# falcon-computing/bwa-flow

Hardware: AMD Instinct MI355X
Metric: million reads/sec (2×150 bp PE) end-to-end align; SW-extend GCUPS at 1/2/4/8 MI355X (higher is better)
Workload: dtype int32

## Files before the change

### bwa-flow_amd/csrc/capi.hip

```cpp
#include <hip/hip_runtime.h>
#include <string.h>

#include <algorithm>
#include <chrono>
#include <cstdio>
#include <mutex>
#include <new>
#include <string>
#include <thread>
#include <vector>

#include "batch_host.h"
#include "ctx.h"
#include "engine.h"
#include "regpost.h"

using namespace bwagpu;

namespace {


__global__ void side_probe_spin(uint64_t ticks) {
  const uint64_t t0 = __builtin_amdgcn_s_memrealtime();
  while (__builtin_amdgcn_s_memrealtime() - t0 < ticks) __builtin_amdgcn_s_sleep(8);
// ... 114 lines not shown
  if (hipGetDeviceCount(&n) != hipSuccess || n <= 0) return BWAGPU_E_NODEVICE;
  if (device < 0 || device >= n) return BWAGPU_E_NODEVICE;
  bwagpu_ctx_t* ctx = new (std::nothrow) bwagpu_ctx_t();
  if (!ctx) return BWAGPU_E_NOMEM;
  std::string why;
  if (!make_opt(opt, &ctx->opt, &why)) {
    delete ctx;
    return BWAGPU_E_INVAL;
  }
  ctx->device = device;
  ctx->opt_b = opt->b;
  ctx->ext_form = set_ext_form(-1);
  ctx->ext_short = ext_short_default();
  ctx->ext_short_fill = ext_short_fill_default();
  ctx->light_pack = light_pack_default();
  *made = ctx;
  HIPC(hipSetDevice(device), "hipSetDevice");
  HIPC(hipMalloc(&ctx->d_ann_off, sizeof(int64_t) * bns->n_seqs), "hipMalloc(ann_offset)");
  HIPC(hipMalloc(&ctx->d_ann_len, sizeof(int32_t) * bns->n_seqs), "hipMalloc(ann_len)");
  HIPC(hipMemcpy(ctx->d_ann_off, bns->ann_offset, sizeof(int64_t) * bns->n_seqs, hipMemcpyHostToDevice),
       "upload ann_offset");
  HIPC(hipMemcpy(ctx->d_ann_len, bns->ann_len, sizeof(int32_t) * bns->n_seqs, hipMemcpyHostToDevice),
       "upload ann_len");
  for (auto& s : ctx->slot) {
    HIPC(hipEventCreate(&s.ev0), "hipEventCreate");
    HIPC(hipEventCreate(&s.ev1), "hipEventCreate");
    HIPC(hipEventCreate(&s.ev2), "hipEventCreate");
    HIPC(hipEventCreate(&s.ev3), "hipEventCreate");
  }
  ctx->ref.l_pac = bns->l_pac;
// ... 138 lines not shown
  HIPC(s.d_heavy.get(a.heavy, nr), "hipMalloc(heavy)");
  HIPC(s.d_redo.get(a.redo, nr), "hipMalloc(redo)");
  HIPC(s.d_rbits.get(a.rbits, nr / 32 + 1), "hipMalloc(rbits)");
  HIPC(s.d_desc.get(a.rdesc, nr), "hipMalloc(desc)");
  HIPC(s.d_schain.get(a.seedchain, ns), "hipMalloc(seedchain)");
  HIPC(s.d_hinfo.get(a.hinfo, nr), "hipMalloc(hinfo)");
  HIPC(s.d_cov.get(a.cov, ns), "hipMalloc(cov)");
  HIPC(s.d_hflag.get(a.hflag, ns), "hipMalloc(hflag)");
  HIPC(s.d_colent.get(a.colent, ns), "hipMalloc(colent)");
  HIPC(s.d_longc.get(a.longc, nc), "hipMalloc(longc)");
  HIPC(s.d_qh.get(a.qh, kQHWords), "hipMalloc(qh)");
  HIPC(s.d_sorth.get(a.sorth, kSortWords), "hipMalloc(sorth)");
  HIPC(s.d_stasks.get(a.stasks, n_tasks), "hipMalloc(stasks)");
  HIPC(s.d_ftask.get(a.ftask, n_tasks), "hipMalloc(ftask)");
  HIPC(s.d_ftaskR.get(a.ftaskR, n_tasks), "hipMalloc(ftaskR)");
  HIPC(s.d_mat.get(a.mat, (size_t)std::max<int64_t>(1 << 20, 16 * (int64_t)ns)), "hipMalloc(mat)");
  a.mat_words = (int64_t)(s.d_mat.cap / sizeof(uint64_t));
  static const int ext_prefetch = [] {
    const char* e = getenv("BWAGPU_EXT_PREFETCH");
    return e ? std::max(0, atoi(e)) : 0;
  }();
  a.ext_prefetch = ext_prefetch;
  static const int risky_first = [] {
    const char* e = getenv("BWAGPU_LIGHT_RISKY_FIRST");
    return e && e[0] == '1';
  }();
  a.risky_first = risky_first;
  static const int emu_strict = [] {
    const char* e = getenv("BWAGPU_EMU_STRICT");
    return !(e && e[0] == '0');
// ... 514 lines not shown
  if (k == BWAGPU_NUM_SLOTS || !ctx->dev_scratch[k].d_ctr.p) return fail(ctx, BWAGPU_E_INVAL, "no device-entry batch on this stream");
  HIPC(hipStreamSynchronize(st), "hipStreamSynchronize");
  int32_t c[SPC_WORDS];
  HIPC(hipMemcpy(c, ctx->dev_scratch[k].d_ctr.p, sizeof c, hipMemcpyDeviceToHost), "hipMemcpy(ctr)");
  out[0] = c[SPC_SHORT_N];
  for (int r = 0; r < 2; ++r) {
    const int l = r * kSpecBins;
    out[1 + 4 * r] = c[SPC_LCNT + l];
    out[2 + 4 * r] = c[SPC_LLONG + l];
    out[3 + 4 * r] = c[SPC_RCNT + l];
    out[4 + 4 * r] = c[SPC_RLONG + l];
  }
  return BWAGPU_OK;
}

int bwagpu_ctx_row_bound(bwagpu_ctx_t* ctx, int on) {
  if (!ctx) return BWAGPU_E_INVAL;
  const int prev = ctx->opt.row_bound;
  if (on >= 0) ctx->opt.row_bound = on ? 1 : 0;
  return prev;
}

int bwagpu_debug_ext_kernel(bwagpu_ctx_t* ctx, int32_t lq_max) {
  if (!ctx || lq_max < 1 || lq_max > BWAGPU_MAX_READ_LEN) return BWAGPU_E_INVAL;
  return ext_kernel_for(ctx->opt, ctx->ext_form, tb_bytes_for(ctx->opt, lq_max));
}

int bwagpu_prof_start(bwagpu_ctx_t* ctx, int max_launches) {
  if (!ctx || max_launches < 0) return BWAGPU_E_INVAL;
  HIPC(hipSetDevice(ctx->device), "hipSetDevice");
// ... 51 lines not shown
```

### bwa-flow_amd/csrc/ctx.h

```cpp
#pragma once
#include <hip/hip_runtime.h>
#include <stdint.h>

#include <algorithm>
#include <atomic>
#include <chrono>
#include <mutex>
#include <string>
#include <type_traits>
#include <vector>

#include "bwagpu.h"
#include "chain.h"
#include "engine.h"
#include "rescue.h"
#include "seed.h"
#include "stage_host.h"
#include "task_host.h"

namespace bwagpu {

inline std::atomic<int64_t> g_live_bufs{0}, g_live_bytes{0};

template <bool kPinned>
// ... 35 lines not shown
  }
  template <class T>
  T* as() const { return (T*)p; }
};
using DevBuf = GrowBuf<false>;
using HostBuf = GrowBuf<true>;
static_assert(!std::is_copy_constructible<DevBuf>::value, "a copy would free the buffer twice");

struct Slot {
  hipStream_t stream = nullptr;
  std::once_flag stream_once;
  hipError_t stream_err = hipSuccess;
  hipEvent_t ev0 = nullptr, ev1 = nullptr, ev2 = nullptr, ev3 = nullptr;
  DevBuf d_in, d_win, d_srt, d_prog, d_desc, d_out, d_n, d_stats, d_lists, d_counts;
  DevBuf d_cread, d_ext, d_tasks, d_ctr, d_regpos, d_skipf, d_heavy, d_redo, d_rbits;
  DevBuf d_schain, d_hinfo, d_mat, d_cov, d_hflag, d_colent, d_qh, d_longc, d_sorth, d_stasks, d_ftask, d_ftaskR;
  SpecStreams spec;
  bool side_chosen = false;
  HostBuf h_in, h_out, h_n, h_stats;
  HostBuf h_dense, h_off;
  DevBuf d_off;
  size_t in_rco = 0, in_cso = 0;
  bool slot_view = false;
  bool busy = false;
  bool has_results = false;
  bool kept = false;
  std::vector<int32_t> keep_rco, keep_cso;
  int32_t n_reads = 0, n_chains = 0, n_seeds = 0;
  std::chrono::steady_clock::time_point t_submit;
  bwagpu_stats_t last{};
  int64_t h2d = 0, d2h = 0;
// ... 30 lines not shown
  using Slot = bwagpu::Slot;
  int device = 0;
  std::mutex side_mu;
  std::vector<hipStream_t> callers, side_graveyard;
  bwagpu::DevOpt opt{};
  bwagpu::DevRef ref{};
  bool own_pac = false;
  void* d_pac = nullptr;
  int64_t* d_ann_off = nullptr;
  int32_t* d_ann_len = nullptr;
  int watchdog_ms = 10000;
  int ext_form = 0;
  int ext_short = 0;
  int light_pack = 0;
  int ext_short_fill = 0;
  Slot slot[BWAGPU_NUM_SLOTS];
  hipStream_t dev_stream[BWAGPU_NUM_SLOTS] = {};
  Slot dev_scratch[BWAGPU_NUM_SLOTS];
  DevBuf ex_tasks, ex_list, ex_q, ex_t, ex_res, ex_stats;
  DevBuf a2_tasks, a2_q, a2_t, a2_out, a2_scratch, a2_lists, a2_counts, a2_boff;
  DevBuf r2_tasks, r2_q, r2_out, r2_cig, r2_md, r2_lists, r2_z, r2_stats;
  DevBuf r2d_keys, r2d_lists, r2d_tab, r2d_z, r2d_sums;
  HostBuf r2d_htab;
  hipEvent_t r2d_done = nullptr, r2d_ev[2] = {};
  bool r2d_pending = false, r2d_timing = false, r2d_timed = false;
  double r2d_wait_ms = 0, r2d_call_ms = 0;
  int32_t r2d_jobs = 0;
  static constexpr int kA2Streams = 4;
  hipStream_t a2_st[kA2Streams] = {};
  hipEvent_t a2_fork = nullptr, a2_join[kA2Streams] = {};
// ... 198 lines not shown
```

### bwa-flow_amd/csrc/engine.h

```cpp
#pragma once
#include <hip/hip_runtime.h>
#include <stdint.h>

#include "bwagpu.h"
#include "bwagpu_debug.h"
#include "pure.h"
#include "spec_plan.h"

namespace bwagpu {

struct ReadDesc {
  int64_t qoff;
  int32_t rd;
  int32_t lq;
  int32_t c0;
  int32_t nch;
  int32_t s0;
  int32_t ns;
};

struct ChainWin {
  int64_t lo, hi;
};

// ... 69 lines not shown
  SPC_CNT = 0,
  SPC_HEAVY_N = 16,
  SPC_SEL_CUR = 17,
  SPC_REDO_N = 20,
  SPC_SPEC64 = 24,
  SPC_MISS = 26,
  SPC_MATW64 = 28,
  SPC_HCOLS = 30,
  SPC_LONG_N = 31,
  SPC_LCNT = 64,
  SPC_RCNT = 73,
  SPC_LIGHT_CUR = 82,
  SPC_LLONG = 84,
  SPC_RLONG = 93,
  SPC_SHORT_N = 102,
  SPC_WORDS = 128
};
constexpr int kQHStride = 32;
constexpr int kQHShort = 2 * kSpecRounds * kSpecBins * 8 * kQHStride;
constexpr int kQHWords = 2 * kQHShort;
constexpr int kSortKeys = 1024;
constexpr int kSortWordsR = kSpecRounds * 2 * kSortKeys;
constexpr int kSortWords = 2 * kSortWordsR;
__host__ __device__ inline size_t spec_list_off(int list, int n_chains, int n_seeds) {
  const int round = list / kSpecBins, bin = list % kSpecBins;
  return round == 0 ? (size_t)bin * n_chains
                    : (size_t)kSpecBins * n_chains + ((size_t)(round - 1) * kSpecBins + bin) * n_seeds;
}
struct FatTask {
  int64_t rbeg, qoff;
  int32_t pos;
  int32_t dlo, dhi;
  uint32_t qls;
};
static_assert(sizeof(FatTask) == 32, "FatTask layout");
static_assert(BWAGPU_MAX_READ_LEN < 1024, "FatTask packs qbeg / len / lq in 10 bits each");
struct SpecArgs {
  int lq_bound;
  ChainWin* win;
  int32_t* chain_read;
  bwagpu_seed_t* prog;
  SeedExt* ext;
  int2* tasks;
  int32_t* ctr;
  int32_t* regpos;
  int32_t* skipf;
  int32_t* heavy;
  int32_t* redo;
  uint32_t* rbits;
  ReadDesc* rdesc;
  int32_t* seedchain;
  int4* hinfo;
  int32_t* colent;
  int32_t* longc;
  uint64_t* mat;
  int64_t mat_words;
  int32_t* cov;
  int32_t* hflag;
  int32_t* qh;
  int32_t* sorth;
  int2* stasks;
  FatTask* ftask;
  FatTask* ftaskR;
  int risky_first;
  int emu_strict;
  int light_pack;
  int ext_prefetch;
  bwagpu_alnreg_t* out;
  int32_t* out_n;
  int64_t* stats;
};
struct SpecStreams {
  hipStream_t side = nullptr;
  hipEvent_t fork = nullptr, join = nullptr;
  hipEvent_t* pool = nullptr;
  int pool_n = 0;
  int* pool_used = nullptr;
  int form = 0;
  int short_q = 0;
  int short_fill = 0;
};
int set_ext_form(int form);
int ext_short_default();
int ext_short_fill_default();
int light_pack_default();
int ext_kernel_for(const DevOpt& o, int form, int tb_bytes);
hipError_t launch_spec_clear(const SpecArgs& a, int n_reads, int n_seeds, hipStream_t st);
hipError_t launch_spec_chain2aln(const DevOpt& o, const DevRef& ref, const DevBatch& b, const SpecArgs& a,
                                 int tb_bytes, int lq_max, hipStream_t st, const SpecStreams& ss);
size_t spec_select_lds(int tb_bytes);
int spec_redo_cap(int tb_bytes);

struct StreamTask {
  bwagpu_seed_t s;
  int64_t lo, hi;
  int64_t qoff;
// ... 24 lines not shown
```

### bwa-flow_amd/csrc/spec.hip

```cpp
#include "spec_dev.h"

namespace bwagpu {

__device__ uint32_t* g_trace = nullptr;
hipError_t set_trace_spec(void* p) { return hipMemcpyToSymbol(HIP_SYMBOL(g_trace), &p, sizeof(p)); }


__global__ void __launch_bounds__(256) spec_chain_kernel(DevOpt o, DevRef ref, DevBatch b, SpecArgs a) {
  sel_prio();
  const int c = blockIdx.x * blockDim.x + threadIdx.x;
  bool task = false, longc = false;
  int bin = 0, s0 = 0;
  if (c < b.n_chains) {
    const int rd = a.chain_read[c];
    s0 = b.chain_seed_off[c];
    const int ns = b.chain_seed_off[c + 1] - s0;
    const int lq = (int)(b.seq_off[rd + 1] - b.seq_off[rd]);
    if (ns <= 0) {
      a.win[c] = ChainWin{0, 0};
    } else {
      int64_t wlo = ref.l_pac << 1, whi = 0;
      longc = ns > kOrderLane;
      if (!longc) {
        uint64_t key[kOrderLane];
// ... 1965 lines not shown

#ifndef BWAGPU_EXT_SHORT_Q_DEFAULT
#define BWAGPU_EXT_SHORT_Q_DEFAULT 63
#endif
int ext_short_default() {
  static const int q = [] {
    const char* e = getenv("BWAGPU_EXT_SHORT_Q");
    const int v = e && e[0] ? atoi(e) : BWAGPU_EXT_SHORT_Q_DEFAULT;
    return std::min(std::max(v, 0), kShortQMax);
  }();
  return q;
}
#ifndef BWAGPU_EXT_SHORT_FILL_DEFAULT
#define BWAGPU_EXT_SHORT_FILL_DEFAULT 150
#endif
int ext_short_fill_default() {
  static const int f = [] {
    const char* e = getenv("BWAGPU_EXT_SHORT_FILL");
    return std::min(std::max(e && e[0] ? atoi(e) : BWAGPU_EXT_SHORT_FILL_DEFAULT, 0), 100000);
  }();
  return f;
}


static void launch_sort(const ExtBin& k, const ExtRound& r, int bin0, int nbins, int short_q) {
  if (k.phased) launch_side_sort(r, bin0, nbins, short_q);
  else launch_task_sort(r, bin0, nbins);
}
static void launch_ext_bin(const ExtBin& k, const ExtRound& r, int list, const ExtPlan& p, int short_fill) {
  if (k.family == SIDE4) launch_side_bin(k, r, list, p, short_fill);
  else launch_task_bin(k, r, list, p.quad);
}

static void launch_ext_round(const DevOpt& o, const DevRef& ref, const DevBatch& b, const SpecArgs& a, int round,
                             int tb_bytes, int lq_max, hipStream_t st, const SpecStreams& ss) {
  const int l = round * kSpecBins;
  const bool bin1 = lq_max > kSpecBinLen[0], bin2 = lq_max > kSpecBinLen[1];
  const ExtPlan plan = ext_plan(o, ss.form, tb_bytes, ss.short_q);
  const ExtRound r{o, ref, b, a, round, tb_bytes, st};
  if (!bin1 || plan.bin[0].phased == plan.bin[1].phased) {
    launch_sort(plan.bin[0], r, 0, bin1 ? 2 : 1, plan.short_q);
  } else {
    launch_sort(plan.bin[0], r, 0, 1, plan.short_q);
    launch_sort(plan.bin[1], r, 1, 1, 0);
  }
  const bool prof = ss.pool && *ss.pool_used + 2 <= ss.pool_n;
  if (prof) (void)hipEventRecord(ss.pool[*ss.pool_used], st);
  launch_ext_bin(plan.bin[0], r, l + 0, plan, ss.short_fill);
  if (prof) {
    (void)hipEventRecord(ss.pool[*ss.pool_used + 1], st);
    *ss.pool_used += 2;
  }
  if (!bin1) return;
  launch_ext_bin(plan.bin[1], r, l + 1, plan, ss.short_fill);
  if (bin2) launch_task_long(r, l + 2);
}

hipError_t launch_spec_chain2aln(const DevOpt& o, const DevRef& ref, const DevBatch& b, const SpecArgs& a,
                                 int tb_bytes, int lq_max, hipStream_t st, const SpecStreams& ss) {
// ... 51 lines not shown
```

### bwa-flow_amd/csrc/spec_dev.h

```cpp
#pragma once
#include "ksw_dev.h"

namespace bwagpu {

__device__ __forceinline__ void sel_prio() { __builtin_amdgcn_s_setprio(3); }

__host__ __device__ inline int64_t tri_off(int k) {
  if (k <= 1) return 0;
  const int64_t q = (k - 1) >> 6;
  return 32 * q * (q + 1) + (int64_t)(k - 1 - 64 * q) * (q + 1);
}

template <int G = 32>
__device__ __forceinline__ void fill_two_half(uint8_t* tbl, int64_t x0l, int nl, uint8_t* tbr, int64_t x0r, int nr,
                                              const DevRef& ref) {
  const int r = (int)(threadIdx.x & (G - 1));
  const int64_t two1 = (ref.l_pac << 1) - 1;
  const int n = max(nl, nr);
  for (int base = 0; base < n; base += 4 * G) {
    uint32_t raw[8];
    int sh[8], kk[8];
    bool rev[8];
#pragma unroll
    for (int m = 0; m < 8; ++m) {
// ... 140 lines not shown
  const int lq = (int)(b.seq_off[rd + 1] - f.qoff);
  f.qls = (uint32_t)sd.qbeg | (uint32_t)sd.len << 10 | (uint32_t)lq << 20;
  return f;
}


struct ExtRound {
  const DevOpt& o;
  const DevRef& ref;
  const DevBatch& b;
  const SpecArgs& a;
  int round, tb_bytes;
  hipStream_t st;
};
int ext2_grid(int nb, bool packed);
void launch_side_sort(const ExtRound& r, int bin0, int nbins, int short_q);
void launch_side_bin(const ExtBin& k, const ExtRound& r, int list, const ExtPlan& p, int short_fill);
constexpr int ext_key(int family, int g, int pmax, bool k8) { return ((family * 64 + g) * 32 + pmax) * 2 + (k8 ? 1 : 0); }

}
```

### bwa-flow_amd/csrc/spec_side.hip

```cpp
#include "spec_dev.h"

namespace bwagpu {

__device__ __forceinline__ int side_key(int qlen) { return 255 - min(qlen, 255); }

__global__ void __launch_bounds__(256) spec_sort2_count(DevBatch b, SpecArgs a, int round, int bin0) {
  sel_prio();
  __shared__ int hist[2][256];
  __shared__ int tot[2];
  const int bin = bin0 + (int)blockIdx.y;
  const int list = round * kSpecBins + bin;
  int32_t* ghL = a.sorth + (round * 2 + bin) * kSortKeys;
  int32_t* ghR = ghL + kSortWordsR;
  for (int k = threadIdx.x; k < 2 * 256; k += 256) hist[k >> 8][k & 255] = 0;
  if (threadIdx.x < 2) tot[threadIdx.x] = 0;
  __syncthreads();
  const int n = __hip_atomic_load(&a.ctr[SPC_CNT + list], __ATOMIC_RELAXED, __HIP_MEMORY_SCOPE_AGENT);
  const int2* tl = a.tasks + spec_list_off(list, b.n_chains, b.n_seeds);
  const int chunk = (n + (int)gridDim.x - 1) / (int)gridDim.x;
  const int i0 = (int)blockIdx.x * chunk, i1 = min(n, i0 + chunk);
  for (int i = i0 + (int)threadIdx.x; i < i1; i += 256) {
    const FatTask f = fat_task(b, a, tl[i]);
    const int qb = (int)(f.qls & 1023u), ln = (int)((f.qls >> 10) & 1023u), lq = (int)(f.qls >> 20);
    const int qr = lq - qb - ln;
    if (qb > 0) atomicAdd(&hist[0][side_key(qb)], 1);
    if (qr > 0) atomicAdd(&hist[1][side_key(qr)], 1);
  }
  __syncthreads();
  for (int k = threadIdx.x; k < 2 * 256; k += 256) {
    const int c = hist[k >> 8][k & 255];
    if (c) {
      atomicAdd((k >> 8) ? &ghR[k & 255] : &ghL[k & 255], c);
      atomicAdd(&tot[k >> 8], c);
    }
  }
  __syncthreads();
  if (threadIdx.x < 2 && tot[threadIdx.x])
    atomicAdd(&a.ctr[(threadIdx.x ? SPC_RCNT : SPC_LCNT) + list], tot[threadIdx.x]);
}

__global__ void __launch_bounds__(256) spec_sort2_scan(SpecArgs a, int round, int bin0, int nbins, int short_q) {
// ... 7 lines not shown
  __syncthreads();
  for (int o = 1; o < 256; o <<= 1) {
    const int x = t >= o ? part[t - o] : 0;
    __syncthreads();
    part[t] += x;
    __syncthreads();
  }
  gh[t] = part[t] - v;
  if (short_q > 0 && bin == 0 && t == side_key(short_q))
    a.ctr[(side ? SPC_RLONG : SPC_LLONG) + round * kSpecBins + bin] = part[t] - v;
}

__global__ void __launch_bounds__(256) spec_sort2_scatter(DevOpt o, DevBatch b, SpecArgs a, int round, int bin0) {
  sel_prio();
  __shared__ int cnt[2][256];
  const int bin = bin0 + (int)blockIdx.y;
  const int list = round * kSpecBins + bin;
  int32_t* ghL = a.sorth + (round * 2 + bin) * kSortKeys;
  int32_t* ghR = ghL + kSortWordsR;
  for (int k = threadIdx.x; k < 2 * 256; k += 256) cnt[k >> 8][k & 255] = 0;
  __syncthreads();
  const int n = __hip_atomic_load(&a.ctr[SPC_CNT + list], __ATOMIC_RELAXED, __HIP_MEMORY_SCOPE_AGENT);
  const size_t off = spec_list_off(list, b.n_chains, b.n_seeds);
  const int2* tl = a.tasks + off;
  FatTask* foL = a.ftask + off;
  FatTask* foR = a.ftaskR + off;
  const int chunk = (n + (int)gridDim.x - 1) / (int)gridDim.x;
  const int i0 = (int)blockIdx.x * chunk, i1 = min(n, i0 + chunk);
  constexpr int kPer = 8;
  int kl[kPer], kr[kPer], rl[kPer], rr[kPer];
  FatTask ft[kPer];
  for (int base = i0; base < i1; base += 256 * kPer) {
#pragma unroll
    for (int m = 0; m < kPer; ++m) {
      const int i = base + m * 256 + (int)threadIdx.x;
      kl[m] = kr[m] = -1;
      if (i < i1) {
        ft[m] = fat_task(b, a, tl[i]);
        const int qb = (int)(ft[m].qls & 1023u), ln = (int)((ft[m].qls >> 10) & 1023u), lq = (int)(ft[m].qls >> 20);
        const int qr = lq - qb - ln;
        if (qb > 0) {
          kl[m] = side_key(qb);
          rl[m] = atomicAdd(&cnt[0][kl[m]], 1);
        }
        if (qr > 0) {
          kr[m] = side_key(qr);
          rr[m] = atomicAdd(&cnt[1][kr[m]], 1);
        }
        if (qb == 0 && qr == 0) {
          SeedExt e;
          e.rb = ft[m].rbeg;
          e.re = ft[m].rbeg + ln;
          e.qb = 0;
          e.qe = lq;
          e.score = e.truesc = ln * o.a;
          e.w = o.w;
          e.cells = e.rows = 0;
          e.calls = 1;
          a.ext[ft[m].pos] = e;
        }
      }
    }
    __syncthreads();
    for (int k = threadIdx.x; k < 2 * 256; k += 256) {
      const int c = cnt[k >> 8][k & 255];
      cnt[k >> 8][k & 255] = c ? atomicAdd((k >> 8) ? &ghR[k & 255] : &ghL[k & 255], c) : 0;
    }
    __syncthreads();
#pragma unroll
    for (int m = 0; m < kPer; ++m) {
      if (kl[m] >= 0) foL[cnt[0][kl[m]] + rl[m]] = ft[m];
      if (kr[m] >= 0) foR[cnt[1][kr[m]] + rr[m]] = ft[m];
    }
    __syncthreads();
    for (int k = threadIdx.x; k < 2 * 256; k += 256) cnt[k >> 8][k & 255] = 0;
    __syncthreads();
  }
}

struct SideTask {
  int64_t rbeg, qoff, rb;
  int32_t pos, dlo, dhi, qbeg, len, lq;
  int32_t tt, score, h0, truesc, qb, aw0, cells, rows, calls, pad_;
};
static_assert(sizeof(SideTask) <= 96, "SideTask layout");
typedef __attribute__((address_space(3))) SideTask LdsS;
#define SIDE_FIELDS(X) X(rbeg) X(qoff) X(rb) X(pos) X(dlo) X(dhi) X(qbeg) X(len) X(lq) X(tt) X(score) X(h0) \
  X(truesc) X(qb) X(aw0) X(cells) X(rows) X(calls)
__device__ __forceinline__ void spark(LdsS* p, const SideTask& t) {
#define X(f) p->f = t.f;
  SIDE_FIELDS(X)
#undef X
// ... 306 lines not shown
        atomicAdd(reinterpret_cast<unsigned long long*>(a.ctr + SPC_SPEC64), (unsigned long long)cells_s);
      }
    }
  }
#ifdef BWAGPU_OCC_DIAG
  if ((threadIdx.x & 63) == 0) {
    for (int k = 0; k < 8; ++k) atomicAdd(reinterpret_cast<unsigned long long*>(a.ctr + 32) + k, occ[k]);
    for (int k = 0; k < 4; ++k) atomicAdd(reinterpret_cast<unsigned long long*>(a.ctr + 48) + k, tw[k]);
  }
#endif
  if ((threadIdx.x & (G - 1)) == 0 && spec_cells)
    atomicAdd(reinterpret_cast<unsigned long long*>(a.ctr + SPC_SPEC64), (unsigned long long)spec_cells);
}


void launch_side_sort(const ExtRound& r, int bin0, int nbins, int short_q) {
  hipLaunchKernelGGL(spec_sort2_count, dim3(256, nbins), dim3(256), 0, r.st, r.b, r.a, r.round, bin0);
  hipLaunchKernelGGL(spec_sort2_scan, dim3(2 * nbins), dim3(256), 0, r.st, r.a, r.round, bin0, nbins, short_q);
  hipLaunchKernelGGL(spec_sort2_scatter, dim3(256, nbins), dim3(256), 0, r.st, r.o, r.b, r.a, r.round, bin0);
}

template <int G, int PMAX, bool K8>
static void launch_side_pair(const ExtRound& r, int list, const ExtPlan& p, int short_fill) {
  const size_t lds = (size_t)(kBlock / 64) * p.wave_lds;
  const int nb = resident_blocks(spec_side4_kernel<G, PMAX, K8, false>, lds);
  const int gr = r.round == 2 ? std::min(nb, 64) : std::min(nb, ext2_grid(1 << 30, true));
  if (!(G == 16 && K8)) short_fill = 0;
  hipLaunchKernelGGL((spec_side4_kernel<G, PMAX, K8, false>), dim3(gr), dim3(kBlock), lds, r.st, r.o, r.ref, r.b, r.a,
                     list, r.tb_bytes, (int)p.wave_lds, p.short_q, p.tb_short, short_fill);
  hipLaunchKernelGGL((spec_side4_kernel<G, PMAX, K8, true>), dim3(gr), dim3(kBlock), lds, r.st, r.o, r.ref, r.b, r.a,
                     list, r.tb_bytes, (int)p.wave_lds, p.short_q, p.tb_short, short_fill);
// ... 13 lines not shown
```

### bwa-flow_amd/python/bwagpu/abi.py

```python
from __future__ import annotations

import ctypes as C
import os

import numpy as np

HERE = os.path.dirname(os.path.abspath(__file__))
PKG_ROOT = os.path.normpath(os.path.join(HERE, "..", ".."))
REPO_ROOT = os.path.normpath(os.path.join(PKG_ROOT, ".."))
LIB_DIR = os.path.join(PKG_ROOT, "lib")

ABI_VERSION = 1
OK, E_INVAL, E_NOMEM, E_DEVICE, E_HANG, E_RESULTS, E_UNSUPPORTED, E_NODEVICE = range(8)
ERR_NAMES = {
    OK: "OK", E_INVAL: "E_INVAL", E_NOMEM: "E_NOMEM", E_DEVICE: "E_DEVICE", E_HANG: "E_HANG",
    E_RESULTS: "E_RESULTS", E_UNSUPPORTED: "E_UNSUPPORTED", E_NODEVICE: "E_NODEVICE",
}
MAX_READ_LEN = 1023
NUM_SLOTS = 4

SEED_DTYPE = np.dtype([("rbeg", "<i8"), ("qbeg", "<i4"), ("len", "<i4"), ("score", "<i4"),
                       ("pad", "<i4")])
ALNREG_DTYPE = np.dtype([
    ("rb", "<i8"), ("re", "<i8"), ("qb", "<i4"), ("qe", "<i4"), ("rid", "<i4"), ("score", "<i4"),
# ... 171 lines not shown
    "bwagpu_debug_occupancy": (C.c_int, [_VP, _VP, _VP]),
    "bwagpu_debug_spec_ext": (C.c_int, [_VP, _VP, _VP, C.c_int32]),
    "bwagpu_prof_read": (C.c_int, [_VP, C.POINTER(C.c_double), C.POINTER(C.c_int32)]),
    "bwagpu_prof_intervals": (C.c_int, [_VP, _VP, _VP, C.c_int32, C.POINTER(C.c_int32)]),
    "bwagpu_set_bwt": (C.c_int, [_VP, C.POINTER(BwtC)]),
    "bwagpu_debug_seed_budget": (C.c_int, [_VP, C.c_int32]),
    "bwagpu_debug_sup_shift": (C.c_int, [_VP, C.c_int32]),
    "bwagpu_set_device_read_len": (C.c_int, [_VP, C.c_int32]),
    "bwagpu_debug_ext_form": (C.c_int, [C.c_int]),
    "bwagpu_ctx_ext_form": (C.c_int, [_VP, C.c_int]),
    "bwagpu_ctx_ext_short": (C.c_int, [_VP, C.c_int]),
    "bwagpu_ctx_ext_short_fill": (C.c_int, [_VP, C.c_int]),
    "bwagpu_ctx_light_pack": (C.c_int, [_VP, C.c_int]),
    "bwagpu_debug_spec_short": (C.c_int, [_VP, _VP, _VP]),
    "bwagpu_ctx_row_bound": (C.c_int, [_VP, C.c_int]),
    "bwagpu_debug_ext_kernel": (C.c_int, [_VP, C.c_int32]),
    "bwagpu_streams_concurrent": (C.c_int, [_VP, _VP]),
    "bwagpu_bwt_sa": (C.c_int, [_VP, C.c_int64, _VP, _VP]),
    "bwagpu_sw_stream": (C.c_int, [_VP, _VP, C.c_int64, _VP, C.c_int32, C.POINTER(C.c_int32)]),
    "bwagpu_collect_intv": (C.c_int, [_VP, C.POINTER(SeedOpt), C.c_int32, _VP, _VP, C.c_int32, _VP, C.c_int64,
                                       _VP]),
    "bwagpu_set_alt": (C.c_int, [_VP, _VP]),
    "bwagpu_seqs2chains": (C.c_int, [_VP, C.POINTER(SeedOpt), C.POINTER(ChainOpt), C.c_int32, _VP, _VP, C.c_int32,
                                      C.POINTER(ChainsC)]),
    "bwagpu_seqs2regions": (C.c_int, [_VP, C.POINTER(SeedOpt), C.POINTER(ChainOpt), C.c_int32, _VP, _VP, _VP,
                                       C.POINTER(_VP), C.POINTER(C.c_int64)]),
    "bwagpu_regs_post": (C.c_int, [_VP, C.POINTER(PostOpt), C.c_int32, C.c_int64, C.c_int32, _VP, _VP, _VP, _VP,
                                    _VP]),
    "bwagpu_regs_post_device": (C.c_int, [_VP, C.POINTER(PostOpt), C.c_int32, C.c_int64, C.POINTER(BatchC), _VP,
                                           _VP, _VP, _VP]),
# ... 24 lines not shown

def load() -> C.CDLL:
    global _lib
    if _lib is not None:
        return _lib
    p = lib_path()
    if os.environ.get("BWAGPU_NO_TORCH") != "1":
        try:
            import torch
        except Exception:
            pass
    if not os.path.exists(p):
        raise RuntimeError(f"bwagpu: HIP engine library missing at {p}; run __graft_entry__.build()")
    lib = C.CDLL(p)
    for name, (res, args) in PROTOS.items():
        if (name.startswith("bwagpu_debug_") or name == "bwagpu_ctx_light_pack") and not hasattr(lib, name):
            continue
        fn = getattr(lib, name)
        fn.restype = res
        fn.argtypes = args
    if lib.bwagpu_abi_version() != ABI_VERSION:
        raise RuntimeError("bwagpu: ABI version mismatch")
    _lib = lib
    return lib


def opt_from_dict(d: dict) -> Opt:
    o = Opt()
    for k in ("a", "b", "o_del", "e_del", "o_ins", "e_ins", "pen_clip5", "pen_clip3", "w", "zdrop"):
        setattr(o, k, int(d[k]))
    mat = d.get("mat")
# ... 19 lines not shown
```

### bwa-flow_amd/python/bwagpu/engine.py

```python
from __future__ import annotations

import ctypes as C
from dataclasses import dataclass

import numpy as np

from . import abi


class BwaGpuError(RuntimeError):
    def __init__(self, code: int, msg: str):
        super().__init__(f"{abi.ERR_NAMES.get(code, code)}: {msg}")
        self.code = code


def _ptr(a: np.ndarray | None):
    return None if a is None or a.size == 0 else a.ctypes.data_as(C.c_void_p)


@dataclass
class Batch:
    seq_off: np.ndarray
    seq: np.ndarray
    read_chain_off: np.ndarray
# ... 277 lines not shown
            raise BwaGpuError(k, "debug_ext_kernel")
        return self.EXT_KERNELS[k]

    def ext_form(self, form: int = -1) -> int:
        return self.lib.bwagpu_ctx_ext_form(self.ctx, int(form))

    def ext_short(self, q: int = -1) -> int:
        return self.lib.bwagpu_ctx_ext_short(self.ctx, int(q))

    def ext_short_fill(self, percent: int = -1) -> int:
        return self.lib.bwagpu_ctx_ext_short_fill(self.ctx, int(percent))

    def light_pack(self, on: int = -1) -> int:
        return self.lib.bwagpu_ctx_light_pack(self.ctx, int(on))

    def row_bound(self, on: int = -1) -> int:
        return self.lib.bwagpu_ctx_row_bound(self.ctx, int(on))

    def set_device_read_len(self, max_len: int):
        self._check(self.lib.bwagpu_set_device_read_len(self.ctx, int(max_len)), "set_device_read_len")

    def sup_shift(self, shift: int):
        self._check(self.lib.bwagpu_debug_sup_shift(self.ctx, shift), "sup_shift")

    def seed_budget(self, budget: int):
        self._check(self.lib.bwagpu_debug_seed_budget(self.ctx, budget), "seed_budget")

    def collect_intv(self, seq_off: np.ndarray, seq: np.ndarray, min_seed_len: int = 19, split_width: int = 10,
                     max_mem_intv: int = 20, split_factor: float = 1.5, max_per_read: int = 256,
                     out_cap: int | None = None, out: np.ndarray | None = None):
# ... 230 lines not shown
```

### include/bwagpu_debug.h

```cpp
#ifndef BWAGPU_DEBUG_H
#define BWAGPU_DEBUG_H
#include "bwagpu.h"

#ifdef __cplusplus
extern "C" {
#endif

int bwagpu_debug_seed_budget(bwagpu_ctx_t *ctx, int32_t budget);

int bwagpu_debug_sup_shift(bwagpu_ctx_t *ctx, int32_t shift);

int bwagpu_debug_set_trace(bwagpu_ctx_t *ctx, void *dev_ptr);
int bwagpu_debug_fail_wait(bwagpu_ctx_t *ctx, int after_n_waits, int code);
int bwagpu_debug_live_buffers(int64_t *n, int64_t *bytes);

int bwagpu_prof_start(bwagpu_ctx_t *ctx, int max_launches);
int bwagpu_debug_spec_counters(bwagpu_ctx_t *ctx, void *stream, int64_t *out);
int bwagpu_debug_occupancy(bwagpu_ctx_t *ctx, void *stream, int64_t *out);
int bwagpu_debug_spec_ext(bwagpu_ctx_t *ctx, void *stream, void *host_out, int32_t n);
int bwagpu_prof_read(bwagpu_ctx_t *ctx, double *total_ms, int32_t *launches);
int bwagpu_debug_ext_form(int form);
int bwagpu_ctx_ext_form(bwagpu_ctx_t *ctx, int form);
int bwagpu_ctx_ext_short(bwagpu_ctx_t *ctx, int q);
int bwagpu_ctx_ext_short_fill(bwagpu_ctx_t *ctx, int percent);
int bwagpu_ctx_light_pack(bwagpu_ctx_t *ctx, int on);
int bwagpu_debug_spec_short(bwagpu_ctx_t *ctx, void *stream, int64_t *out);
int bwagpu_ctx_row_bound(bwagpu_ctx_t *ctx, int on);
int bwagpu_debug_ext_kernel(bwagpu_ctx_t *ctx, int32_t lq_max);
int bwagpu_streams_concurrent(void *a, void *b);
int bwagpu_debug_rescue_drop(bwagpu_ctx_t *ctx, int32_t k);
int bwagpu_debug_rescue_times(bwagpu_ctx_t *ctx, double *out);
int bwagpu_debug_reg2aln_times(bwagpu_ctx_t *ctx, double *out);
int bwagpu_prof_intervals(bwagpu_ctx_t *ctx, double *start_ms, double *end_ms, int32_t max, int32_t *n);

#ifdef __cplusplus
}
#endif
#endif
```

Measured before the change: 64.55.

## Settle gap-free seed extensions with an ungapped pre-scan before banded SW

Adds a pre-pass kernel that scans each seed side without gaps, using packed 16-base loads of query and reference. Where the side provably cannot benefit from a gap (mismatch penalty stays below the cheapest gap open), the result is computed directly. Those sides are then kept out of the sort and banded Smith-Waterman lists. This cuts DP work for easy extensions, at the cost of an extra kernel launch, a per-task record buffer, and correctness relying on the bound that the ungapped result equals the banded one. The path is on by default when row_bound is set.

```diff
diff --git a/bwa-flow_amd/csrc/capi.hip b/bwa-flow_amd/csrc/capi.hip
--- a/bwa-flow_amd/csrc/capi.hip
+++ b/bwa-flow_amd/csrc/capi.hip
@@ -152,6 +152,7 @@
   ctx->ext_short = ext_short_default();
   ctx->ext_short_fill = ext_short_fill_default();
   ctx->light_pack = light_pack_default();
+  ctx->ungapped = ungapped_default();
   *made = ctx;
   HIPC(hipSetDevice(device), "hipSetDevice");
   HIPC(hipMalloc(&ctx->d_ann_off, sizeof(int64_t) * bns->n_seqs), "hipMalloc(ann_offset)");
@@ -320,6 +321,8 @@
   HIPC(s.d_stasks.get(a.stasks, n_tasks), "hipMalloc(stasks)");
   HIPC(s.d_ftask.get(a.ftask, n_tasks), "hipMalloc(ftask)");
   HIPC(s.d_ftaskR.get(a.ftaskR, n_tasks), "hipMalloc(ftaskR)");
+  a.ung = nullptr;
+  if (ctx->ungapped && ctx->opt.row_bound) HIPC(s.d_ung.get(a.ung, n_tasks), "hipMalloc(ung)");
   HIPC(s.d_mat.get(a.mat, (size_t)std::max<int64_t>(1 << 20, 16 * (int64_t)ns)), "hipMalloc(mat)");
   a.mat_words = (int64_t)(s.d_mat.cap / sizeof(uint64_t));
   static const int ext_prefetch = [] {
@@ -864,6 +867,35 @@
   return BWAGPU_OK;
 }
 
+int bwagpu_ctx_ungapped(bwagpu_ctx_t* ctx, int on) {
+  if (!ctx) return BWAGPU_E_INVAL;
+  const int prev = ctx->ungapped;
+  if (on >= 0) ctx->ungapped = on ? 1 : 0;
+  return prev;
+}
+
+int bwagpu_debug_spec_ungapped(bwagpu_ctx_t* ctx, void* stream, int64_t* out) {
+  if (!ctx || !out) return BWAGPU_E_INVAL;
+  hipStream_t st = nullptr;
+  if (int rc = entry_stream(ctx, stream, &st)) return rc;
+  int k = 0;
+  while (k < BWAGPU_NUM_SLOTS && ctx->dev_stream[k] != st) ++k;
+  if (k == BWAGPU_NUM_SLOTS || !ctx->dev_scratch[k].d_ctr.p) return fail(ctx, BWAGPU_E_INVAL, "no device-entry batch on this stream");
+  HIPC(hipStreamSynchronize(st), "hipStreamSynchronize");
+  int32_t c[SPC_WORDS];
+  HIPC(hipMemcpy(c, ctx->dev_scratch[k].d_ctr.p, sizeof c, hipMemcpyDeviceToHost), "hipMemcpy(ctr)");
+  for (int r = 0; r < kSpecRounds; ++r) {
+    out[4 * r + 0] = c[SPC_UNG_N + r];
+    out[4 * r + 1] = c[SPC_UNG_Q + r];
+    out[4 * r + 2] = out[4 * r + 3] = 0;
+    for (int bin = 0; bin < kSpecBins; ++bin) {
+      out[4 * r + 2] += c[SPC_LCNT + r * kSpecBins + bin];
+      out[4 * r + 3] += c[SPC_RCNT + r * kSpecBins + bin];
+    }
+  }
+  return BWAGPU_OK;
+}
+
 int bwagpu_ctx_row_bound(bwagpu_ctx_t* ctx, int on) {
   if (!ctx) return BWAGPU_E_INVAL;
   const int prev = ctx->opt.row_bound;
diff --git a/bwa-flow_amd/csrc/ctx.h b/bwa-flow_amd/csrc/ctx.h
--- a/bwa-flow_amd/csrc/ctx.h
+++ b/bwa-flow_amd/csrc/ctx.h
@@ -73,7 +73,7 @@
   hipEvent_t ev0 = nullptr, ev1 = nullptr, ev2 = nullptr, ev3 = nullptr;
   DevBuf d_in, d_win, d_srt, d_prog, d_desc, d_out, d_n, d_stats, d_lists, d_counts;
   DevBuf d_cread, d_ext, d_tasks, d_ctr, d_regpos, d_skipf, d_heavy, d_redo, d_rbits;
-  DevBuf d_schain, d_hinfo, d_mat, d_cov, d_hflag, d_colent, d_qh, d_longc, d_sorth, d_stasks, d_ftask, d_ftaskR;
+  DevBuf d_schain, d_hinfo, d_mat, d_cov, d_hflag, d_colent, d_qh, d_longc, d_sorth, d_stasks, d_ftask, d_ftaskR, d_ung;
   SpecStreams spec;
   bool side_chosen = false;
   HostBuf h_in, h_out, h_n, h_stats;
@@ -134,6 +134,7 @@
   int ext_short = 0;
   int light_pack = 0;
   int ext_short_fill = 0;
+  int ungapped = 1;
   Slot slot[BWAGPU_NUM_SLOTS];
   hipStream_t dev_stream[BWAGPU_NUM_SLOTS] = {};
   Slot dev_scratch[BWAGPU_NUM_SLOTS];
diff --git a/bwa-flow_amd/csrc/engine.h b/bwa-flow_amd/csrc/engine.h
--- a/bwa-flow_amd/csrc/engine.h
+++ b/bwa-flow_amd/csrc/engine.h
@@ -6,6 +6,7 @@
 #include "bwagpu_debug.h"
 #include "pure.h"
 #include "spec_plan.h"
+#include "ungapped.h"
 
 namespace bwagpu {
 
@@ -107,6 +108,8 @@
   SPC_LLONG = 84,
   SPC_RLONG = 93,
   SPC_SHORT_N = 102,
+  SPC_UNG_N = 103,
+  SPC_UNG_Q = 106,
   SPC_WORDS = 128
 };
 constexpr int kQHStride = 32;
@@ -128,6 +131,13 @@
 };
 static_assert(sizeof(FatTask) == 32, "FatTask layout");
 static_assert(BWAGPU_MAX_READ_LEN < 1024, "FatTask packs qbeg / len / lq in 10 bits each");
+struct UngRec {
+  struct Side {
+    int32_t ok;
+    UngappedSide s;
+  } side[2];
+};
+static_assert(sizeof(UngRec) == 32, "UngRec layout");
 struct SpecArgs {
   int lq_bound;
   ChainWin* win;
@@ -155,6 +165,7 @@
   int2* stasks;
   FatTask* ftask;
   FatTask* ftaskR;
+  UngRec* ung;
   int risky_first;
   int emu_strict;
   int light_pack;
@@ -173,6 +184,7 @@
   int short_q = 0;
   int short_fill = 0;
 };
+int ungapped_default();
 int set_ext_form(int form);
 int ext_short_default();
 int ext_short_fill_default();
diff --git a/bwa-flow_amd/csrc/spec.hip b/bwa-flow_amd/csrc/spec.hip
--- a/bwa-flow_amd/csrc/spec.hip
+++ b/bwa-flow_amd/csrc/spec.hip
@@ -2003,6 +2003,13 @@
 #ifndef BWAGPU_EXT_SHORT_FILL_DEFAULT
 #define BWAGPU_EXT_SHORT_FILL_DEFAULT 150
 #endif
+int ungapped_default() {
+  static const int on = [] {
+    const char* e = getenv("BWAGPU_UNGAPPED");
+    return !(e && e[0] == '0');
+  }();
+  return on;
+}
 int ext_short_fill_default() {
   static const int f = [] {
     const char* e = getenv("BWAGPU_EXT_SHORT_FILL");
@@ -2012,8 +2019,8 @@
 }
 
 
-static void launch_sort(const ExtBin& k, const ExtRound& r, int bin0, int nbins, int short_q) {
-  if (k.phased) launch_side_sort(r, bin0, nbins, short_q);
+static void launch_sort(const ExtBin& k, const ExtRound& r, int bin0, int nbins, int short_q, int short_fill) {
+  if (k.phased) launch_side_sort(r, bin0, nbins, short_q, short_fill);
   else launch_task_sort(r, bin0, nbins);
 }
 static void launch_ext_bin(const ExtBin& k, const ExtRound& r, int list, const ExtPlan& p, int short_fill) {
@@ -2028,10 +2035,10 @@
   const ExtPlan plan = ext_plan(o, ss.form, tb_bytes, ss.short_q);
   const ExtRound r{o, ref, b, a, round, tb_bytes, st};
   if (!bin1 || plan.bin[0].phased == plan.bin[1].phased) {
-    launch_sort(plan.bin[0], r, 0, bin1 ? 2 : 1, plan.short_q);
+    launch_sort(plan.bin[0], r, 0, bin1 ? 2 : 1, plan.short_q, ss.short_fill);
   } else {
-    launch_sort(plan.bin[0], r, 0, 1, plan.short_q);
-    launch_sort(plan.bin[1], r, 1, 1, 0);
+    launch_sort(plan.bin[0], r, 0, 1, plan.short_q, ss.short_fill);
+    launch_sort(plan.bin[1], r, 1, 1, 0, ss.short_fill);
   }
   const bool prof = ss.pool && *ss.pool_used + 2 <= ss.pool_n;
   if (prof) (void)hipEventRecord(ss.pool[*ss.pool_used], st);
diff --git a/bwa-flow_amd/csrc/spec_dev.h b/bwa-flow_amd/csrc/spec_dev.h
--- a/bwa-flow_amd/csrc/spec_dev.h
+++ b/bwa-flow_amd/csrc/spec_dev.h
@@ -178,7 +178,7 @@
   hipStream_t st;
 };
 int ext2_grid(int nb, bool packed);
-void launch_side_sort(const ExtRound& r, int bin0, int nbins, int short_q);
+void launch_side_sort(const ExtRound& r, int bin0, int nbins, int short_q, int short_fill);
 void launch_side_bin(const ExtBin& k, const ExtRound& r, int list, const ExtPlan& p, int short_fill);
 constexpr int ext_key(int family, int g, int pmax, bool k8) { return ((family * 64 + g) * 32 + pmax) * 2 + (k8 ? 1 : 0); }
 
diff --git a/bwa-flow_amd/csrc/spec_side.hip b/bwa-flow_amd/csrc/spec_side.hip
--- a/bwa-flow_amd/csrc/spec_side.hip
+++ b/bwa-flow_amd/csrc/spec_side.hip
@@ -3,6 +3,152 @@
 namespace bwagpu {
 
 __device__ __forceinline__ int side_key(int qlen) { return 255 - min(qlen, 255); }
+
+
+struct UngSide {
+  const uint8_t* rd;
+  int64_t x0;
+  int p0, d, qlen, lq;
+};
+struct UngPass {
+  uint64_t qw[2], tw;
+  int64_t fa, b0;
+  int base, last, ws;
+  bool fast, rev;
+};
+__device__ __forceinline__ UngPass ung_load(const UngSide& s, const DevRef& ref, int base) {
+  UngPass p;
+  p.base = base;
+  p.last = min(base + 15, s.qlen - 1);
+  p.fast = false;
+  if (base >= s.qlen) return p;
+  const int64_t two1 = (ref.l_pac << 1) - 1, pac_bytes = (ref.l_pac >> 2) + 1;
+  const int64_t xa = s.x0 + (int64_t)s.d * base, xb = s.x0 + (int64_t)s.d * p.last;
+  p.rev = xa >= ref.l_pac;
+  p.fa = p.rev ? two1 - xa : xa;
+  const int64_t fb = p.rev ? two1 - xb : xb;
+  p.fast = s.lq >= 16 && pac_bytes >= 8 && (xb >= ref.l_pac) == p.rev;
+  if (p.fast) {
+    p.ws = min(max(min(s.p0 + s.d * base, s.p0 + s.d * (base + 15)), 0), s.lq - 16);
+    p.b0 = min(min(p.fa, fb) >> 2, pac_bytes - 8);
+    __builtin_memcpy(p.qw, s.rd + p.ws, 16);
+    __builtin_memcpy(&p.tw, ref.pac + p.b0, 8);
+  }
+  return p;
+}
+__device__ __forceinline__ void ung_eat(const UngSide& s, const DevRef& ref, const UngPass& p, const int8_t* mat,
+                                        int max_mat, UngappedScan& sc) {
+  if (p.base >= s.qlen) return;
+  if (p.fast) {
+#pragma unroll
+    for (int m = 0; m < 16; ++m)
+      if (p.base + m <= p.last) {
+        const int k = s.p0 + s.d * (p.base + m) - p.ws;
+        const int qv = (int)(p.qw[k >> 3] >> ((k & 7) * 8)) & 255;
+        const int64_t fm = p.fa + (p.rev ? -s.d : s.d) * m;
+        const int byte = (int)(p.tw >> (((fm >> 2) - p.b0) * 8)) & 255;
+        const int bse = (byte >> ((~fm & 3) << 1)) & 3;
+        sc.step(p.base + m, mat[(p.rev ? 3 - bse : bse) * 5 + min(qv, 4)], max_mat);
+      }
+  } else {
+    for (int j = p.base; j <= p.last; ++j)
+      sc.step(j, mat[pac_base2(ref.pac, ref.l_pac, s.x0 + (int64_t)s.d * j) * 5 + min((int)s.rd[s.p0 + s.d * j], 4)],
+              max_mat);
+  }
+}
+
+__global__ void __launch_bounds__(256) spec_ungapped_kernel(DevOpt o, DevRef ref, DevBatch b, SpecArgs a, int round,
+                                                            int bin0, int keep_short) {
+  sel_prio();
+  __shared__ int8_t mat[25];
+  if (threadIdx.x < 25) mat[threadIdx.x] = o.mat[threadIdx.x];
+  __syncthreads();
+  const int bin = bin0 + (int)blockIdx.y;
+  const int list = round * kSpecBins + bin;
+  const int n = __hip_atomic_load(&a.ctr[SPC_CNT + list], __ATOMIC_RELAXED, __HIP_MEMORY_SCOPE_AGENT);
+  const size_t off = spec_list_off(list, b.n_chains, b.n_seeds);
+  const int2* tl = a.tasks + off;
+  const int oe_min = ungapped_oe_min(o.o_del, o.e_del, o.o_ins, o.e_ins);
+  const int keep = bin == 0 ? keep_short : 0;
+  const int chunk = (n + (int)gridDim.x - 1) / (int)gridDim.x;
+  const int i0 = (int)blockIdx.x * chunk, i1 = min(n, i0 + chunk);
+  for (int k = 2 * i0 + (int)threadIdx.x; k < 2 * i1; k += 256) {
+    const int i = k >> 1, right = k & 1;
+    const FatTask f = fat_task(b, a, tl[i]);
+    const int qb = (int)(f.qls & 1023u), ln = (int)((f.qls >> 10) & 1023u), lq = (int)(f.qls >> 20);
+    const int64_t xr = f.rbeg + ln;
+    const int qlen = right ? lq - qb - ln : qb;
+    const int tlen = right ? (int)(f.rbeg + f.dhi - xr) : f.dlo;
+    UngRec::Side rec{0, {0, 0, 0}};
+    if (qlen > keep && ungapped_band_ok(o.w) &&
+        ungapped_call_ok(qlen, tlen, ln * o.a, o.w, o.zdrop, o.max_mat, oe_min)) {
+      UngSide sd;
+      sd.rd = b.seq + f.qoff;
+      sd.p0 = right ? qb + ln : qb - 1;
+      sd.d = right ? 1 : -1;
+      sd.x0 = right ? xr : f.rbeg - 1;
+      sd.qlen = qlen;
+      sd.lq = lq;
+      UngappedScan sc;
+      for (int base = 0; base < qlen && !sc.dead(oe_min); base += 16)
+        ung_eat(sd, ref, ung_load(sd, ref, base), mat, o.max_mat, sc);
+      if (!sc.dead(oe_min)) rec = UngRec::Side{1, sc.side()};
+    }
+    a.ung[off + i].side[right] = rec;
+  }
+}
+
+struct SideLists {
+  bool cl, cr, in_l, in_r;
+};
+__device__ __forceinline__ SideLists side_lists(const SpecArgs& a, size_t slot, int qb, int qr) {
+  SideLists s{false, false, qb > 0, qr > 0};
+  if (a.ung) {
+    s.cl = qb > 0 && a.ung[slot].side[0].ok;
+    s.in_l = qb > 0 && !s.cl;
+    s.cr = qr > 0 && a.ung[slot].side[1].ok && !s.in_l;
+    s.in_r = qr > 0 && !s.cr;
+  }
+  return s;
+}
+
+__device__ __forceinline__ SeedExt settle_sides(const DevOpt& o, const FatTask& f, const UngRec& u, bool right) {
+  const int qb = (int)(f.qls & 1023u), ln = (int)((f.qls >> 10) & 1023u), lq = (int)(f.qls >> 20);
+  const int qr = lq - qb - ln;
+  SeedExt e;
+  int calls = 0;
+  e.rb = f.rbeg;
+  e.qb = 0;
+  e.score = e.truesc = ln * o.a;
+  if (qb > 0) {
+    const UngappedOut x = ungapped_result(ln * o.a, qb, u.side[0].s);
+    const bool local = x.gscore <= 0 || x.gscore <= x.score - o.pen_clip5;
+    e.rb = f.rbeg - (local ? x.tle : x.gtle);
+    e.qb = local ? qb - x.qle : 0;
+    e.score = x.score;
+    e.truesc = local ? x.score : x.gscore;
+    ++calls;
+  }
+  e.re = f.rbeg + ln;
+  e.qe = lq;
+  if (right) {
+    const int h0 = e.score;
+    const UngappedOut x = ungapped_result(h0, qr, u.side[1].s);
+    const bool local = x.gscore <= 0 || x.gscore <= x.score - o.pen_clip3;
+    e.qe = local ? qb + ln + x.qle : lq;
+    e.re = f.rbeg + ln + (local ? x.tle : x.gtle);
+    e.score = x.score;
+    e.truesc += (local ? x.score : x.gscore) - h0;
+    ++calls;
+  } else if (qr > 0) {
+    e.re = 0;
+    e.qe = 0;
+  }
+  e.w = o.w;
+  e.cells = e.rows = 0;
+  e.calls = calls + (right || qr == 0 ? 1 : 0);
+  return e;
+}
 
 __global__ void __launch_bounds__(256) spec_sort2_count(DevBatch b, SpecArgs a, int round, int bin0) {
   sel_prio();
@@ -16,15 +162,17 @@
   if (threadIdx.x < 2) tot[threadIdx.x] = 0;
   __syncthreads();
   const int n = __hip_atomic_load(&a.ctr[SPC_CNT + list], __ATOMIC_RELAXED, __HIP_MEMORY_SCOPE_AGENT);
-  const int2* tl = a.tasks + spec_list_off(list, b.n_chains, b.n_seeds);
+  const size_t off = spec_list_off(list, b.n_chains, b.n_seeds);
+  const int2* tl = a.tasks + off;
   const int chunk = (n + (int)gridDim.x - 1) / (int)gridDim.x;
   const int i0 = (int)blockIdx.x * chunk, i1 = min(n, i0 + chunk);
   for (int i = i0 + (int)threadIdx.x; i < i1; i += 256) {
     const FatTask f = fat_task(b, a, tl[i]);
     const int qb = (int)(f.qls & 1023u), ln = (int)((f.qls >> 10) & 1023u), lq = (int)(f.qls >> 20);
     const int qr = lq - qb - ln;
-    if (qb > 0) atomicAdd(&hist[0][side_key(qb)], 1);
-    if (qr > 0) atomicAdd(&hist[1][side_key(qr)], 1);
+    const SideLists sl = side_lists(a, off + i, qb, qr);
+    if (sl.in_l) atomicAdd(&hist[0][side_key(qb)], 1);
+    if (sl.in_r) atomicAdd(&hist[1][side_key(qr)], 1);
   }
   __syncthreads();
   for (int k = threadIdx.x; k < 2 * 256; k += 256) {
@@ -62,11 +210,13 @@
 __global__ void __launch_bounds__(256) spec_sort2_scatter(DevOpt o, DevBatch b, SpecArgs a, int round, int bin0) {
   sel_prio();
   __shared__ int cnt[2][256];
+  __shared__ int ung[2];
   const int bin = bin0 + (int)blockIdx.y;
   const int list = round * kSpecBins + bin;
   int32_t* ghL = a.sorth + (round * 2 + bin) * kSortKeys;
   int32_t* ghR = ghL + kSortWordsR;
   for (int k = threadIdx.x; k < 2 * 256; k += 256) cnt[k >> 8][k & 255] = 0;
+  if (threadIdx.x < 2) ung[threadIdx.x] = 0;
   __syncthreads();
   const int n = __hip_atomic_load(&a.ctr[SPC_CNT + list], __ATOMIC_RELAXED, __HIP_MEMORY_SCOPE_AGENT);
   const size_t off = spec_list_off(list, b.n_chains, b.n_seeds);
@@ -87,25 +237,22 @@
         ft[m] = fat_task(b, a, tl[i]);
         const int qb = (int)(ft[m].qls & 1023u), ln = (int)((ft[m].qls >> 10) & 1023u), lq = (int)(ft[m].qls >> 20);
         const int qr = lq - qb - ln;
-        if (qb > 0) {
+        const SideLists sl = side_lists(a, off + i, qb, qr);
+        if (sl.in_l) {
           kl[m] = side_key(qb);
           rl[m] = atomicAdd(&cnt[0][kl[m]], 1);
         }
-        if (qr > 0) {
+        if (sl.in_r) {
           kr[m] = side_key(qr);
           rr[m] = atomicAdd(&cnt[1][kr[m]], 1);
         }
-        if (qb == 0 && qr == 0) {
-          SeedExt e;
-          e.rb = ft[m].rbeg;
-          e.re = ft[m].rbeg + ln;
-          e.qb = 0;
-          e.qe = lq;
-          e.score = e.truesc = ln * o.a;
-          e.w = o.w;
-          e.cells = e.rows = 0;
-          e.calls = 1;
-          a.ext[ft[m].pos] = e;
+        if (!sl.in_l) {
+          if (qb > 0 || !sl.in_r)
+            a.ext[ft[m].pos] = settle_sides(o, ft[m], sl.cl || sl.cr ? a.ung[off + i] : UngRec{}, sl.cr);
+          if (sl.cl || sl.cr) {
+            atomicAdd(&ung[0], (sl.cl ? 1 : 0) + (sl.cr ? 1 : 0));
+            atomicAdd(&ung[1], (sl.cl ? qb : 0) + (sl.cr ? qr : 0));
+          }
         }
       }
     }
@@ -124,6 +271,8 @@
     for (int k = threadIdx.x; k < 2 * 256; k += 256) cnt[k >> 8][k & 255] = 0;
     __syncthreads();
   }
+  if (threadIdx.x < 2 && ung[threadIdx.x])
+    atomicAdd(&a.ctr[(threadIdx.x ? SPC_UNG_Q : SPC_UNG_N) + round], ung[threadIdx.x]);
 }
 
 struct SideTask {
@@ -460,7 +609,10 @@
 }
 
 
-void launch_side_sort(const ExtRound& r, int bin0, int nbins, int short_q) {
+void launch_side_sort(const ExtRound& r, int bin0, int nbins, int short_q, int short_fill) {
+  if (r.a.ung)
+    hipLaunchKernelGGL(spec_ungapped_kernel, dim3(1024, nbins), dim3(256), 0, r.st, r.o, r.ref, r.b, r.a, r.round, bin0,
+                       short_fill == 0 ? short_q : 0);
   hipLaunchKernelGGL(spec_sort2_count, dim3(256, nbins), dim3(256), 0, r.st, r.b, r.a, r.round, bin0);
   hipLaunchKernelGGL(spec_sort2_scan, dim3(2 * nbins), dim3(256), 0, r.st, r.a, r.round, bin0, nbins, short_q);
   hipLaunchKernelGGL(spec_sort2_scatter, dim3(256, nbins), dim3(256), 0, r.st, r.o, r.b, r.a, r.round, bin0);
diff --git a/bwa-flow_amd/csrc/ungapped.h b/bwa-flow_amd/csrc/ungapped.h
--- /dev/null
+++ b/bwa-flow_amd/csrc/ungapped.h
@@ -0,0 +1,68 @@
+#pragma once
+#include <stdint.h>
+
+#ifdef __HIPCC__
+#define BWAGPU_UNG_HD __host__ __device__
+#else
+#define BWAGPU_UNG_HD
+#endif
+
+namespace bwagpu {
+
+struct UngappedSide {
+  int32_t M;
+  int32_t am;
+  int32_t cl;
+};
+
+struct UngappedOut {
+  int32_t score, qle, tle, gtle, gscore, max_off;
+};
+
+BWAGPU_UNG_HD inline int ungapped_oe_min(int o_del, int e_del, int o_ins, int e_ins) {
+  const int d = o_del + e_del, i = o_ins + e_ins;
+  return d < i ? d : i;
+}
+
+BWAGPU_UNG_HD inline bool ungapped_call_ok(int qlen, int tlen, int h0, int w, int zdrop, int max_mat, int oe_min) {
+  return qlen >= 1 && tlen >= qlen && max_mat >= 1 && oe_min >= 1 && h0 >= oe_min && w >= 0 &&
+         (zdrop <= 0 || zdrop >= oe_min);
+}
+BWAGPU_UNG_HD inline bool ungapped_band_ok(int w) { return (w >> 1) + (w >> 2) > 0; }
+
+struct UngappedScan {
+  int c = 0, P = 0, M = 0, am = 0;
+  BWAGPU_UNG_HD void step(int i, int s, int max_mat) {
+    P += max_mat - s;
+    c += s;
+    if (c > M) {
+      M = c;
+      am = i + 1;
+    }
+  }
+  BWAGPU_UNG_HD bool dead(int oe_min) const { return P >= oe_min; }
+  BWAGPU_UNG_HD UngappedSide side() const { return UngappedSide{M, am, c}; }
+};
+
+template <class Score>
+BWAGPU_UNG_HD inline bool ungapped_scan(int qlen, int max_mat, int oe_min, Score score, UngappedSide* u) {
+  UngappedScan sc;
+  for (int i = 0; i < qlen; ++i) {
+    sc.step(i, score(i), max_mat);
+    if (sc.dead(oe_min)) return false;
+  }
+  *u = sc.side();
+  return true;
+}
+
+BWAGPU_UNG_HD inline UngappedOut ungapped_result(int h0, int qlen, const UngappedSide& u) {
+  UngappedOut x;
+  x.score = h0 + u.M;
+  x.qle = x.tle = u.am;
+  x.gscore = h0 + u.cl;
+  x.gtle = qlen;
+  x.max_off = 0;
+  return x;
+}
+
+}
diff --git a/bwa-flow_amd/python/bwagpu/abi.py b/bwa-flow_amd/python/bwagpu/abi.py
--- a/bwa-flow_amd/python/bwagpu/abi.py
+++ b/bwa-flow_amd/python/bwagpu/abi.py
@@ -209,6 +209,8 @@
     "bwagpu_ctx_light_pack": (C.c_int, [_VP, C.c_int]),
     "bwagpu_debug_spec_short": (C.c_int, [_VP, _VP, _VP]),
     "bwagpu_ctx_row_bound": (C.c_int, [_VP, C.c_int]),
+    "bwagpu_ctx_ungapped": (C.c_int, [_VP, C.c_int]),
+    "bwagpu_debug_spec_ungapped": (C.c_int, [_VP, _VP, _VP]),
     "bwagpu_debug_ext_kernel": (C.c_int, [_VP, C.c_int32]),
     "bwagpu_streams_concurrent": (C.c_int, [_VP, _VP]),
     "bwagpu_bwt_sa": (C.c_int, [_VP, C.c_int64, _VP, _VP]),
@@ -263,7 +265,7 @@
         raise RuntimeError(f"bwagpu: HIP engine library missing at {p}; run __graft_entry__.build()")
     lib = C.CDLL(p)
     for name, (res, args) in PROTOS.items():
-        if (name.startswith("bwagpu_debug_") or name == "bwagpu_ctx_light_pack") and not hasattr(lib, name):
+        if (name.startswith("bwagpu_debug_") or name in ("bwagpu_ctx_light_pack", "bwagpu_ctx_ungapped")) and not hasattr(lib, name):
             continue
         fn = getattr(lib, name)
         fn.restype = res
diff --git a/bwa-flow_amd/python/bwagpu/engine.py b/bwa-flow_amd/python/bwagpu/engine.py
--- a/bwa-flow_amd/python/bwagpu/engine.py
+++ b/bwa-flow_amd/python/bwagpu/engine.py
@@ -315,6 +315,9 @@
     def light_pack(self, on: int = -1) -> int:
         return self.lib.bwagpu_ctx_light_pack(self.ctx, int(on))
 
+    def ungapped(self, on: int = -1) -> int:
+        return self.lib.bwagpu_ctx_ungapped(self.ctx, int(on))
+
     def row_bound(self, on: int = -1) -> int:
         return self.lib.bwagpu_ctx_row_bound(self.ctx, int(on))
 
diff --git a/include/bwagpu_debug.h b/include/bwagpu_debug.h
--- a/include/bwagpu_debug.h
+++ b/include/bwagpu_debug.h
@@ -25,6 +25,8 @@
 int bwagpu_ctx_ext_short_fill(bwagpu_ctx_t *ctx, int percent);
 int bwagpu_ctx_light_pack(bwagpu_ctx_t *ctx, int on);
 int bwagpu_debug_spec_short(bwagpu_ctx_t *ctx, void *stream, int64_t *out);
+int bwagpu_ctx_ungapped(bwagpu_ctx_t *ctx, int on);
+int bwagpu_debug_spec_ungapped(bwagpu_ctx_t *ctx, void *stream, int64_t *out);
 int bwagpu_ctx_row_bound(bwagpu_ctx_t *ctx, int on);
 int bwagpu_debug_ext_kernel(bwagpu_ctx_t *ctx, int32_t lq_max);
 int bwagpu_streams_concurrent(void *a, void *b);
diff --git a/tools_dev/ungapped_share.py b/tools_dev/ungapped_share.py
--- /dev/null
+++ b/tools_dev/ungapped_share.py
@@ -0,0 +1,43 @@
+#!/usr/bin/env python3
+import ctypes as C
+import json
+import os
+import sys
+
+import numpy as np
+import torch
+
+REPO = os.path.normpath(os.path.join(os.path.dirname(os.path.abspath(__file__)), ".."))
+sys.path.insert(0, os.path.join(REPO, "bwa-flow_amd", "python"))
+from bwagpu import abi, workload
+from bwagpu.engine import Engine
+
+nb = int(sys.argv[1]) if len(sys.argv) > 1 else 2
+opt, ref, rbs = workload.load_fixture()
+eng = Engine(0, opt, ref.l_pac, ref.ann_offset, ref.ann_len, pac=ref.pac)
+dev = torch.device("cuda:0")
+fields = ("seq_off", "seq", "read_chain_off", "chain_seed_off", "chain_rid", "chain_frac_rep", "seeds")
+out = {"fixture": "c2_refseed", "batches": []}
+for k, rb in enumerate(rbs[:nb]):
+    b = rb.batch
+    t = {f: torch.from_numpy(np.ascontiguousarray(getattr(b, f)).view(np.uint8).copy()).to(dev) for f in fields}
+    regs = torch.zeros(max(b.n_seeds, 1) * 88, dtype=torch.uint8, device=dev)
+    nn = torch.zeros(max(b.n_reads, 1), dtype=torch.int32, device=dev)
+    c = abi.BatchC()
+    c.n_reads, c.n_chains, c.n_seeds = b.n_reads, b.n_chains, b.n_seeds
+    c.seq_bytes = int(b.seq_off[-1])
+    for f in fields:
+        setattr(c, f, t[f].data_ptr())
+    st = torch.cuda.current_stream()
+    eng.chain2aln_device(c, regs.data_ptr(), nn.data_ptr(), None, st.cuda_stream)
+    torch.cuda.synchronize()
+    ctr = np.zeros(12, np.int64)
+    assert eng.lib.bwagpu_debug_spec_ungapped(eng.ctx, C.c_void_p(st.cuda_stream), ctr.ctypes.data_as(C.c_void_p)) == 0
+    ok = rb.check(regs.cpu().numpy().view(abi.ALNREG_DTYPE)[:b.n_seeds], nn.cpu().numpy()[:b.n_reads])
+    rounds = {}
+    for r, name in enumerate("AB"):
+        settled, bases, left, right = (int(x) for x in ctr[4 * r:4 * r + 4])
+        rounds[name] = {"settled_sides": settled, "settled_bases": bases, "listed_left": left, "listed_right": right,
+                        "settled_share_of_sides": round(settled / max(settled + left + right, 1), 4)}
+    out["batches"].append({"batch": k, "reads": b.n_reads, "regions_match_reference": bool(ok), "rounds": rounds})
+print(json.dumps(out))
```

Result: faster. 67.45 (median of 6 runs) (+4.5%).
